# mateomarin/two_towers

Measured on AMD Instinct MI355X. Metric: training pairs/sec at global batch=8192, 1/2/4/8 GPUs; MRR@10 match, higher is better.
Workload: dtype bf16; 1 GPU; BASELINE configs[2]: EnhancedTwoTowerModel(300, 256), seq_len 64, batch 8192 per GPU, bf16, hard-negative mining k=5 + margin 0.2, dropout 0.1, Adam; global_batch=8192, seq_len=64, hidden=256, embedding_dim=300, parallelism=dp1, loss=hardneg_margin

## Files before the change

### include/tt_hip.h

```cpp
#ifndef TT_HIP_H
#define TT_HIP_H
#include <stdint.h>

#ifdef __cplusplus
extern "C" {
#endif

#define TT_OK 0
#define TT_EINVAL 1000
#define TT_DT_F32 0
#define TT_DT_BF16 1

const char* tt_version(void);
const char* tt_last_error(void);
int tt_set_option(const char* name, int value);
int tt_get_option(const char* name, int* value);

int tt_embed_gather(int dtype, const void* table, long vocab, int ep, const int32_t* ids, long n,
                    void* out, void* stream);

int tt_pack_rows(int dtype, const float* src, long n, int e, int ep, void* out, void* stream);
typedef struct {
  const float* src;
  const float* src2;
  void* dst;
  int rows, cols, dcols;
  long lds, ldd;
  int dst_bf16;
} tt_pack_job;
int tt_pack_multi(const tt_pack_job* jobs, int njobs, void* stream);

int tt_cast(int dtype, const float* x, long n, void* y, void* stream);

int tt_colsum(const float* x, long rows, int cols, long ld, float* out, int accumulate, void* stream);

typedef struct {
  const void* a[4];
  const void* b[4];
  void* c[4];
  const float* bias[4];
  int bshift[4];
  const void* a_hi[4];
  int a_split;
  uint32_t drop_row0;
} tt_gemm_batch;

int tt_gemm(int dtype, int out_dtype, int a_kouter, int b_kouter, int m, int n, int k,
            const tt_gemm_batch* batch, int nbatch, long lda, long ldb, long ldc, float alpha,
            int beta_accum, int relu, int seq_t, uint32_t drop_seed, float drop_p, int splits,
            float* splitk_ws, void* stream);
long tt_gemm_ws_size(int m, int n, int nbatch, int splits);
int tt_gemm_pick_splits(int m, int n, int k, int nbatch);

typedef struct {
  const void* g;
  const void* whh;
  const float* bhn;
  void* y;
  void* x1;
// ... 136 lines not shown
```

### two_towers_amd/_lib.py

```python
from __future__ import annotations

import contextlib
import ctypes
import os
from ctypes import POINTER, c_float, c_int, c_long, c_uint32, c_void_p

import torch

_HERE = os.path.dirname(os.path.abspath(__file__))
LIB_PATH = os.environ.get("TT_HIP_LIB", os.path.join(_HERE, "lib", "libtt_hip.so"))

DT_F32 = 0
DT_BF16 = 1
TT_EINVAL = 1000


class TTError(RuntimeError):
    pass


class GruTimeoutError(TTError):
    """A column-split GRU forward launch gave up waiting for one of its member workgroups
    (tt_gru_fwd's status word): that launch's outputs are invalid."""


class GemmBatch(ctypes.Structure):
    _fields_ = [
        ("a", c_void_p * 4),
        ("b", c_void_p * 4),
        ("c", c_void_p * 4),
        ("bias", c_void_p * 4),
        ("bshift", c_int * 4),
        ("a_hi", c_void_p * 4),
        ("a_split", c_int),
        ("drop_row0", c_uint32),
    ]


class PackJob(ctypes.Structure):
    _fields_ = [
        ("src", c_void_p),
        ("src2", c_void_p),
        ("dst", c_void_p),
        ("rows", c_int),
        ("cols", c_int),
        ("dcols", c_int),
        ("lds", c_long),
        ("ldd", c_long),
        ("dst_bf16", c_int),
    ]


class GruFwdRec(ctypes.Structure):
    _fields_ = [
        ("g", c_void_p), ("whh", c_void_p), ("bhn", c_void_p), ("y", c_void_p), ("x1", c_void_p),
        ("save", c_void_p), ("hstate", c_void_p), ("dir", c_int), ("drop_seed", c_uint32),
        ("drop_col0", c_int), ("drop_row0", c_uint32),
    ]


class GruInferRec(ctypes.Structure):
    _fields_ = [
        ("g", c_void_p), ("whh", c_void_p), ("bhn", c_void_p), ("y", c_void_p), ("hfinal", c_void_p),
        ("scratch", c_void_p), ("dir", c_int),
# ... 189 lines not shown
```

### two_towers_amd/csrc/tt_api.h

```cpp
#pragma once
#include <hip/hip_runtime.h>
#include <stdio.h>
#include <string.h>

#include "../../include/tt_hip.h"

namespace tt {
void set_error(const char* fmt, ...);

enum Opt {
  OPT_GRU_STEP,
  OPT_GRU_DEPTH,
  OPT_GRU_BWD_ROWS,
  OPT_GRU_BWD_BIG,
  OPT_GRU_BWD_STREAMS,
  OPT_GEMM_PERSIST,
  OPT_GEMM_A3,
  OPT_GEMM_REGSTAGE,
  OPT_GEMM_STREAM_OUT,
  OPT_HN_GEMM,
  OPT_GRU_BWD_PERSIST,
  OPT_GRU_FWD_STEP_ROWS,
  OPT_INFONCE_FLASH,
  OPT_HN_MAP,
// ... 3 lines not shown
  OPT_GRU_XC_SKIP,
  OPT_GRU_XC_SPINS,
  OPT_GRU_BWD_SKEW,
  OPT_GRU_FWD_SKEW,
  OPT_GEMM_BRES,
  OPT_GRU_XC_COOP,
  OPT_GEMM_BUF,
  OPT_GEMM_ORDER,
  OPT_GRU_STEP_RING,
  OPT_GRU_FWD_XS,
  OPT_HN_SCAN_GEMM,
  OPT_GEMM_IEPI,
  OPT_BRES_ROWS,
  OPT_HN_SCAN_V,
  OPT_GEMM_W4,
  OPT_N
};
int opt(Opt o);
int tt_hn_scan_gemm(const void* q, long bq, const void* d, long nd, int h, long label_off, float* cm, long nch,
                    hipStream_t st);
}

#define TT_CHECK_ARG(cond, ...)            \
  do {                                     \
    if (!(cond)) {                         \
      tt::set_error(__VA_ARGS__);          \
      return TT_EINVAL;                    \
    }                                      \
  } while (0)

// ... 26 lines not shown
```

### two_towers_amd/csrc/tt_elem.hip

```cpp
#include <algorithm>

#include "tt_api.h"
#include "tt_common.h"

namespace {

__global__ __launch_bounds__(256) void embed_gather_kernel(const uint4* __restrict__ table, long vocab,
                                                           int cpr, const int32_t* __restrict__ ids,
                                                           long n, uint4* __restrict__ out) {
  const long total = n * cpr;
  for (long e = (long)blockIdx.x * 256 + threadIdx.x; e < total; e += (long)gridDim.x * 256) {
    const long row = e / cpr;
    const int c = (int)(e - row * cpr);
    const int id = ids[row];
    uint4 v = make_uint4(0, 0, 0, 0);
    if (id >= 0 && id < vocab) v = table[(long)id * cpr + c];
    out[e] = v;
  }
}

template <typename T>
__global__ __launch_bounds__(256) void pack_rows_kernel(const float* __restrict__ src, long n, int e, int ep,
                                                        T* __restrict__ out) {
  const long total = n * ep;
// ... 26 lines not shown
    out[c] = accumulate ? out[c] + t : t;
  }
}

__global__ __launch_bounds__(256) void sum_kernel(const float* __restrict__ x, long n, float scale,
                                                  float* __restrict__ out) {
  __shared__ float part[4];
  float s = 0.f;
  for (long i = threadIdx.x; i < n; i += 256) s += x[i];
  s = wave_sum(s);
  if ((threadIdx.x & 63) == 0) part[threadIdx.x >> 6] = s;
  __syncthreads();
  if (threadIdx.x == 0) out[0] = scale * (part[0] + part[1] + part[2] + part[3]);
}

struct PackArgs {
  tt_pack_job j[16];
  long start[17];
  int n;
};
__global__ __launch_bounds__(256) void pack_multi_kernel(PackArgs a) {
  const long total = a.start[a.n];
  for (long i = blockIdx.x * 256L + threadIdx.x; i < total; i += (long)gridDim.x * 256) {
    int k = 0;
    while (k + 1 < a.n && i >= a.start[k + 1]) ++k;
    const tt_pack_job& J = a.j[k];
    const long q = i - a.start[k];
    const int g4 = J.dcols / 4;
    const long r = q / g4;
    const int c = (int)(q - r * g4) * 4;
    float4 v = make_float4(0.f, 0.f, 0.f, 0.f);
    if (c < J.cols) {
      v = *reinterpret_cast<const float4*>(J.src + r * J.lds + c);
      if (J.src2) {
        const float4 w = *reinterpret_cast<const float4*>(J.src2 + r * J.lds + c);
        v.x += w.x; v.y += w.y; v.z += w.z; v.w += w.w;
      }
    }
    if (J.dst_bf16) {
      const uint2 o = make_uint2((uint32_t)f2bf(v.x) | ((uint32_t)f2bf(v.y) << 16),
                                 (uint32_t)f2bf(v.z) | ((uint32_t)f2bf(v.w) << 16));
      *reinterpret_cast<uint2*>(static_cast<bf16_t*>(J.dst) + r * J.ldd + c) = o;
// ... 25 lines not shown
}

extern "C" int tt_pack_rows(int dtype, const float* src, long n, int e, int ep, void* out, void* stream) {
  TT_CHECK_ARG(ep >= e, "tt_pack_rows: ep < e");
  if (n == 0) return 0;
  dim3 g(grid_for(n * ep));
  if (dtype == TT_DT_BF16)
    hipLaunchKernelGGL(pack_rows_kernel<bf16_t>, g, dim3(256), 0, (hipStream_t)stream, src, n, e, ep, (bf16_t*)out);
  else
    hipLaunchKernelGGL(pack_rows_kernel<float>, g, dim3(256), 0, (hipStream_t)stream, src, n, e, ep, (float*)out);
  TT_CHECK_LAUNCH("pack_rows_kernel");
  return 0;
}

extern "C" int tt_pack_multi(const tt_pack_job* jobs, int njobs, void* stream) {
  TT_CHECK_ARG(njobs >= 0 && njobs <= 16 && (njobs == 0 || jobs), "tt_pack_multi: njobs %d not in [0,16]", njobs);
  PackArgs a{};
  a.n = njobs;
  a.start[0] = 0;
  for (int k = 0; k < njobs; ++k) {
    const tt_pack_job& J = jobs[k];
    TT_CHECK_ARG(J.src && J.dst && J.rows >= 0 && J.cols >= 0 && J.dcols >= J.cols, "tt_pack_multi: job %d", k);
    TT_CHECK_ARG(J.cols % 4 == 0 && J.dcols % 4 == 0 && J.lds % 4 == 0 && J.ldd % 4 == 0 && J.lds >= J.cols &&
                     J.ldd >= J.dcols,
                 "tt_pack_multi: job %d: cols, dcols and leading dimensions must be multiples of 4", k);
    const bool src_ok = ((uintptr_t)J.src | (uintptr_t)J.src2) % 16 == 0;
    TT_CHECK_ARG(src_ok && (uintptr_t)J.dst % (J.dst_bf16 ? 8 : 16) == 0, "tt_pack_multi: job %d: misaligned operand", k);
    a.j[k] = J;
    a.start[k + 1] = a.start[k] + (long)J.rows * (J.dcols / 4);
  }
  if (a.start[njobs] == 0) return 0;
  hipLaunchKernelGGL(pack_multi_kernel, dim3(grid_for(a.start[njobs], 256, 4096)), dim3(256), 0, (hipStream_t)stream, a);
  TT_CHECK_LAUNCH("pack_multi_kernel");
  return 0;
}

extern "C" int tt_cast(int dtype, const float* x, long n, void* y, void* stream) {
  if (n == 0) return 0;
  dim3 g(grid_for(n));
  if (dtype == TT_DT_BF16)
    hipLaunchKernelGGL(cast_kernel<bf16_t>, g, dim3(256), 0, (hipStream_t)stream, x, n, (bf16_t*)y);
  else
    hipLaunchKernelGGL(cast_kernel<float>, g, dim3(256), 0, (hipStream_t)stream, x, n, (float*)y);
  TT_CHECK_LAUNCH("cast_kernel");
// ... 22 lines not shown
```

### two_towers_amd/csrc/tt_gemm.hip

```cpp
#include <float.h>
#include <stdarg.h>
#include <stdlib.h>

#include <atomic>
#include <type_traits>

#include "tt_api.h"
#include "tt_gemm_core.h"

namespace tt {
static thread_local char g_err[512];
void set_error(const char* fmt, ...) {
  va_list ap;
  va_start(ap, fmt);
  vsnprintf(g_err, sizeof(g_err), fmt, ap);
  va_end(ap);
}
}

namespace tt {
namespace {
struct OptDef {
  const char* name;
  const char* env;
// ... 4 lines not shown
    {"gru_bwd_rows", "TT_GRU_BWD_ROWS", 0},     {"gru_bwd_big", "TT_GRU_BWD_BIG", 1},
    {"gru_bwd_streams", "TT_GRU_BWD_STREAMS", 2}, {"gemm_persist", "TT_GEMM_PERSIST", 1},
    {"gemm_a3", "TT_GEMM_A3", 1},                 {"gemm_regstage", "TT_GEMM_REGSTAGE", 0},
    {"gemm_stream_out", "TT_GEMM_STREAM_OUT", 1}, {"hn_gemm", "TT_HN_GEMM", 0},
    {"gru_bwd_persist", "TT_GRU_BWD_PERSIST", 1}, {"gru_fwd_step_rows", "TT_GRU_FWD_STEP_ROWS", 0},
    {"infonce_flash", "TT_INFONCE_FLASH", 1},     {"hn_map", "TT_HN_MAP", 2},
    {"gemm_skew", "TT_GEMM_SKEW", 0},             {"gemm_persist_maxk", "TT_GEMM_PERSIST_MAXK", 24},
    {"gru_fwd_xc", "TT_GRU_FWD_XC", 1},           {"gru_xc_skip", "TT_GRU_XC_SKIP", 0},
    {"gru_xc_spins", "TT_GRU_XC_SPINS", 22},      {"gru_bwd_skew", "TT_GRU_BWD_SKEW", 14},
    {"gru_fwd_skew", "TT_GRU_FWD_SKEW", 0},       {"gemm_bres", "TT_GEMM_BRES", 1},
    {"gru_xc_coop", "TT_GRU_XC_COOP", 0},         {"gemm_buf", "TT_GEMM_BUF", 1},
    {"gemm_order", "TT_GEMM_ORDER", 0},           {"gru_step_ring", "TT_GRU_STEP_RING", 4},
    {"gru_fwd_xs", "TT_GRU_FWD_XS", 1},           {"hn_scan_gemm", "TT_HN_SCAN_GEMM", 0},
    {"gemm_iepi", "TT_GEMM_IEPI", 1},             {"bres_rows", "TT_BRES_ROWS", 32},
    {"hn_scan_v", "TT_HN_SCAN_V", 5},             {"gemm_w4", "TT_GEMM_W4", 0},
};
struct OptTable {
  std::atomic<int> v[OPT_N];
  OptTable() {
    for (int i = 0; i < OPT_N; ++i) {
      const char* e = getenv(kOpts[i].env);
      v[i].store(e && *e ? atoi(e) : kOpts[i].dflt, std::memory_order_relaxed);
    }
  }
};
OptTable& opts() {
  static OptTable t;
  return t;
}
int find_opt(const char* name) {
// ... 23 lines not shown
namespace {

struct GemmArgs {
  const void* a[4];
  const void* b[4];
  void* c[4];
  const float* bias[4];
  int bshift[4];
  const void* a_hi[4];
  int a_split;
  long lda, ldb, ldc;
  int M, N, K;
  int splits, kt_per_split;
  float alpha;
  int beta, relu, seq_t;
  uint32_t drop_seed, drop_thresh, drop_row0;
  float drop_inv_keep;
  long part_stride;
  int vec_ok;
  int force_regstage;
  int skew;
  int bias_vec_ok;
  int stream_out;
  int walk_g, walk_x;
  int nbatch;
  float* cm;
  long nch, label_off;
};

constexpr int BM = 128, BN = 128;

// ... 126 lines not shown
      if (gm < g.M && gn < g.N) {
        float v[8];
#pragma unroll
        for (int e = 0; e < 8; ++e) v[e] = L[rl * CLD + cg + e];
        const bool full = gn + 8 <= g.N && g.vec_ok;
        if (partial) {
          float* dst = P + (long)gm * ldc + gn;
          if (full) st8(dst, v);
          else
            for (int e = 0; e < 8 && gn + e < g.N; ++e) dst[e] = v[e];
        } else {
#pragma unroll
          for (int e = 0; e < 8; ++e) {
            float x = v[e] * g.alpha + bv[e];
            if (g.relu) x = fmaxf(x, 0.f);
            if (g.drop_thresh) x *= tt_dropout_scale(g.drop_seed, g.drop_row0 + (uint32_t)gm, gn + e, g.drop_thresh, g.drop_inv_keep);
            v[e] = x;
          }
          TO* dst = C + (long)gm * ldc + gn;
          if (full) {
            if (g.beta) {
              float o[8];
              ld8(dst, o);
#pragma unroll
              for (int e = 0; e < 8; ++e) v[e] += o[e];
            }
            if (g.stream_out)
              st8_sc1(crs, (int)(((long)(gm - m0) * ldc + (gn - n0)) * (long)sizeof(TO)), v, (TO*)nullptr);
            else
              st8(dst, v);
          } else {
// ... 2 lines not shown
              if (g.beta) x += Elt<TO>::ld(dst + e);
              Elt<TO>::st(dst + e, x);
            }
          }
        }
      }
    }
    __syncthreads();
  }
}

template <typename TO>
constexpr int EPI_STORES = sizeof(TO) == 2 ? 16 : 32;

template <typename TO, int MI = -1, int NI = -1>
TT_DEV void epi_direct(const GemmArgs& g, const f32x4 (&acc)[8][4], TO* C, const float* bias, int m0, int n0,
                       int wm, int wn, bool full) {
  constexpr int I0 = MI < 0 ? 0 : 4 * MI, I1 = MI < 0 ? 8 : 4 * MI + 4;
  constexpr int JP0 = NI < 0 ? 0 : NI, JP1 = NI < 0 ? 2 : NI + 1;
  const int lane = threadIdx.x & 63, q = lane >> 4, lr = lane & 15;
  float bv[4][4];
#pragma unroll
  for (int j = 0; j < 4; ++j)
#pragma unroll
    for (int e = 0; e < 4; ++e) bv[j][e] = 0.f;
  if (bias) {
#pragma unroll
    for (int j = 2 * JP0; j < 2 * JP1; ++j) {
      const int c = n0 + wn + 16 * j + 4 * q;
      if (full && g.bias_vec_ok) {
        const float4 b4 = *reinterpret_cast<const float4*>(bias + c);
        bv[j][0] = b4.x; bv[j][1] = b4.y; bv[j][2] = b4.z; bv[j][3] = b4.w;
// ... 3 lines not shown
      }
    }
  }
#ifdef TT_DIAG
  if (g.force_regstage == 9) {
    float sum = 0.f;
#pragma unroll
    for (int i = 0; i < 8; ++i)
#pragma unroll
      for (int j = 0; j < 4; ++j) sum += acc[i][j][0] + acc[i][j][3] + bv[j][0];
    if (sum == 12345.f) C[0] = (TO)0;
    return;
  }
#endif
  const __amdgpu_buffer_rsrc_t crs = tt_rsrc(C + (long)m0 * g.ldc + n0);
  auto fin = [&](float x, float b, int gm, int gn) {
    x = x * g.alpha + b;
    if (g.relu) x = fmaxf(x, 0.f);
    if (g.drop_thresh) x *= tt_dropout_scale(g.drop_seed, g.drop_row0 + (uint32_t)gm, gn, g.drop_thresh, g.drop_inv_keep);
    return x;
  };
  auto put = [&](int gm, int gn, uint4 v) {
#ifdef TT_DIAG
    if (g.force_regstage == 10) {
      *reinterpret_cast<uint4*>(C + (long)(gm & 63) * g.ldc + gn) = v;
      return;
    }
#endif
    const int off = (int)(((long)(gm - m0) * g.ldc + (gn - n0)) * (long)sizeof(TO));
    if (g.stream_out == 2) st16_buf_aux<2>(crs, off, v);
    else if (g.stream_out == 3) st16_buf_aux<17>(crs, off, v);
    else if (g.stream_out) st16_sc1(crs, off, v);
    else *reinterpret_cast<uint4*>(C + (long)gm * g.ldc + gn) = v;
  };
// ... 340 lines not shown
    } else {
      return ttg::KOPlain<T>{B, g.ldb, t.n0, q < qend ? g.N - t.n0 : 0};
    }
  };
#ifdef TT_DIAG
  if constexpr (A3) {
    if (g.force_regstage == 11) {
      f32x4 acc[8][4];
#pragma unroll
      for (int i = 0; i < 8; ++i)
#pragma unroll
        for (int j = 0; j < 4; ++j) acc[i][j] = f32x4{(float)i, (float)j, 1.f, 2.f};
      for (int q = qbeg; q < qend; q += qstep) {
        const TileId t = decode(q);
        const bool full = t.m0 + 256 <= g.M && t.n0 + 256 <= g.N && g.vec_ok;
        epi_direct<TO>(g, acc, static_cast<TO*>(g.c[t.bi]), g.bias[t.bi], t.m0, t.n0, wm, wn, full);
      }
      return;
    }
  }
#endif
  auto la = loader_a(qbeg);
  auto lb = loader_b(qbeg);
  typename L8::template Half<AKO, decltype(la)> pa0, pa1;
  typename L8::template Half<BKO, decltype(lb)> pb0, pb1;
  pa0.init(la, 0, nk, g.K, 0);
  pa1.init(la, 0, nk, g.K, 128);
  pb0.init(lb, 0, nk, g.K, 0);
  pb1.init(lb, 0, nk, g.K, 128);
  if constexpr (A3) {
    pa0.issue(0, base);
// ... 160 lines not shown
      }
      ra_off -= nk;
      rb_off -= nk;
      if constexpr (HN) {
        epi_chunkmax(g, acc, cur_t.m0, cur_t.n0, wm, wn);
        epi_full = __builtin_amdgcn_readfirstlane((int)(cur_t.m0 + 256 <= g.M && cur_t.n0 + 256 <= 64 * g.nch)) != 0;
        continue;
      }
      const bool full = cur_t.m0 + 256 <= g.M && cur_t.n0 + 256 <= g.N && g.vec_ok;
      if constexpr (IEPI) {
        prev_t = cur_t;
        have_prev = true;
        epi_full = __builtin_amdgcn_readfirstlane((int)full) != 0;
        continue;
      }
      epi_direct<TO>(g, acc, static_cast<TO*>(g.c[cur_t.bi]), g.bias[cur_t.bi], cur_t.m0, cur_t.n0, wm, wn, full);
      epi_full = __builtin_amdgcn_readfirstlane((int)full) != 0;
      continue;
    }
    for (int r = 0; r < (A3 ? 0 : nk); ++r, ++git) {
      const int cs = git & 1;
      const uint32_t cur = base + cs * L8::SLOT, nxt = base + (cs ^ 1) * L8::SLOT;
      const char* ia = lds + cs * L8::SLOT + wr * L8::HALF;
      const char* ib = lds + cs * L8::SLOT + (2 + bh) * L8::HALF;
      if (r + 1 == nk) {
        la = loader_a(qn);
        pa0.init(la, 0, nk, g.K, 0);
        pa1.init(la, 0, nk, g.K, 128);
        ra_off = nk;
      }
#pragma unroll
// ... 56 lines not shown
      asm volatile("s_waitcnt lgkmcnt(0)" ::: "memory");
      __builtin_amdgcn_s_barrier();
#pragma unroll
      for (int k = 0; k < 2; ++k) {
        const int rl = rlo + 16 * k;
        const int gm = m0 + p * 32 + rl, gn = n0 + cg;
        if (gm < g.M && gn < g.N) {
          float v[8];
          const float4 x0 = *reinterpret_cast<const float4*>(stg + rl * 256 + cg);
          const float4 x1 = *reinterpret_cast<const float4*>(stg + rl * 256 + cg + 4);
          v[0] = x0.x; v[1] = x0.y; v[2] = x0.z; v[3] = x0.w; v[4] = x1.x; v[5] = x1.y; v[6] = x1.z; v[7] = x1.w;
#pragma unroll
          for (int e = 0; e < 8; ++e) {
            float x = v[e] * g.alpha + bv[e];
            if (g.relu) x = fmaxf(x, 0.f);
            if (g.drop_thresh) x *= tt_dropout_scale(g.drop_seed, g.drop_row0 + (uint32_t)gm, gn + e, g.drop_thresh, g.drop_inv_keep);
            v[e] = x;
          }
          TO* dst = C + (long)gm * g.ldc + gn;
          if (gn + 8 <= g.N && g.vec_ok) {
            if (g.stream_out)
              st8_sc1(crs, (int)(((long)(gm - m0) * g.ldc + (gn - n0)) * (long)sizeof(TO)), v, (TO*)nullptr);
            else
              st8(dst, v);
          } else {
            for (int e = 0; e < 8 && gn + e < g.N; ++e) Elt<TO>::st(dst + e, v[e]);
          }
        }
      }
      __builtin_amdgcn_s_barrier();
    }
// ... 341 lines not shown
  }
  if constexpr (std::is_same<T, bf16_t>::value && std::is_same<TO, bf16_t>::value) {
    if (tt::opt(tt::OPT_GEMM_W4) && !akout && !bkout && !shift && g.splits == 1 && !g.beta && !g.relu &&
        !g.drop_thresh && g.alpha == 1.f && g.force_regstage == 0 && g.M % 256 == 0 && g.N % 256 == 0 && g.K % 64 == 0 &&
        g.K >= 32 && g.vec_ok && g.bias_vec_ok && (g.lda * 2) % 16 == 0 && (g.ldb * 2) % 16 == 0 &&
        256L * g.lda * 2 < (1L << 31) && 256L * g.ldb * 2 < (1L << 31) && 256L * g.ldc * 2 < (1L << 31)) {
      const int ntm = g.M / 256, ntn = g.N / 256;
      if (tt::opt(tt::OPT_GEMM_W4) == 2)
        hipLaunchKernelGGL(gemm_w4<true>, dim3((unsigned)(ntm * ntn * nbatch)), dim3(256), 0, st, g, ntm, ntn);
      else
        hipLaunchKernelGGL(gemm_w4<false>, dim3((unsigned)(ntm * ntn * nbatch)), dim3(256), 0, st, g, ntm, ntn);
      TT_CHECK_LAUNCH("gemm_w4");
      return 0;
    }
  }
  if (dma && persist_ok && !shift && (g.force_regstage == 0 || g.force_regstage >= 9) && g.splits == 1 && !g.beta && nk >= 2 && nk <= tt::opt(tt::OPT_GEMM_PERSIST_MAXK) && t256 >= 512 &&
      use_big(g.M, g.N, t256))
    return launch_persist<T, TO>(akout, bkout, shift, g, (int)t256, buf, st);
  if (dma && g.force_regstage != 2 && use_big(g.M, g.N, t256)) {
    if (tt::opt(tt::OPT_GEMM_A3) && buf)
      return launch_t<T, TO, 256, 256, 2, 4, true, true, true>(akout, bkout, shift, g, t256, st);
    if (tt::opt(tt::OPT_GEMM_A3)) return launch_t<T, TO, 256, 256, 2, 4, true, true>(akout, bkout, shift, g, t256, st);
    return launch_t<T, TO, 256, 256, 2, 4, true>(akout, bkout, shift, g, t256, st);
  }
  const long t128 = (long)tt_ceil_div(g.M, 128) * tt_ceil_div(g.N, 128) * nbatch * g.splits;
  if (dma) return launch_t<T, TO, 128, 128, 2, 2, true>(akout, bkout, shift, g, t128, st);
  return launch_t<T, TO, 128, 128, 2, 2, false>(akout, bkout, shift, g, t128, st);
}

}

// ... 82 lines not shown
    g.a_hi[b] = batch->a_hi[b];
    if (batch->a_split > 0)
      TT_CHECK_ARG(batch->a_hi[b] && (uintptr_t)batch->a_hi[b] % 16 == 0, "tt_gemm: a_hi[%d] null or misaligned", b);
    if (batch->bshift[b] != 0) shift = true;
  }
  TT_CHECK_ARG(!shift || (b_kouter && seq_t > 0), "tt_gemm: bshift needs b_kouter and seq_t");
  TT_CHECK_ARG(batch->a_split >= 0 && (batch->a_split == 0 || (a_kouter && batch->a_split % (16 / esz) == 0)),
               "tt_gemm: a_split %d needs a_kouter and a 16-byte multiple", batch->a_split);
  g.a_split = batch->a_split;
  g.lda = lda; g.ldb = ldb; g.ldc = ldc;
  g.M = m; g.N = n; g.K = k;
  g.alpha = alpha; g.beta = beta_accum; g.relu = relu; g.seq_t = seq_t;
  g.force_regstage = tt::opt(tt::OPT_GEMM_REGSTAGE);
  g.nbatch = nbatch;
  g.skew = tt::opt(tt::OPT_GEMM_SKEW);
  g.drop_seed = drop_seed;
  g.drop_row0 = batch->drop_row0;
  g.drop_thresh = drop_p > 0.f ? (uint32_t)(drop_p * 16777216.0f + 0.5f) : 0u;
  g.drop_inv_keep = drop_p > 0.f ? 1.0f / (1.0f - drop_p) : 1.0f;
  const int nk = tt_ceil_div((long)k * esz, 128);
  if (splits > nk) splits = nk > 0 ? nk : 1;
  g.kt_per_split = nk > 0 ? tt_ceil_div(nk, splits) : 1;
  splits = nk > 0 ? tt_ceil_div(nk, g.kt_per_split) : 1;
  g.splits = splits;
  {
    const int osz = out_dtype == TT_DT_BF16 ? 2 : 4;
    bool ok = (ldc * osz) % 16 == 0;
    for (int b = 0; b < nbatch; ++b) ok = ok && ((uintptr_t)batch->c[b] % 16 == 0);
    g.vec_ok = ok;
    bool bok = true;
    for (int b = 0; b < nbatch; ++b) bok = bok && ((uintptr_t)batch->bias[b] % 16 == 0);
    g.bias_vec_ok = bok;
// ... 34 lines not shown
```

### two_towers_amd/ops.py

```python
from __future__ import annotations

import ctypes
from typing import Sequence

import torch

from . import _lib
from ._lib import GemmBatch, call, dtype_code, ptr, stream_ptr


def _esz(dt: torch.dtype) -> int:
    return 2 if dt == torch.bfloat16 else 4


def pad_cols(e: int, dt: torch.dtype) -> int:
    epc = 128 // _esz(dt)
    return (e + epc - 1) // epc * epc


def gemm(a: Sequence[torch.Tensor], b: Sequence[torch.Tensor], c: Sequence[torch.Tensor], *, m: int, n: int,
         k: int, lda: int, ldb: int, ldc: int, a_kouter: bool, b_kouter: bool, dtype: torch.dtype,
         out_dtype: torch.dtype, bias: Sequence[torch.Tensor | None] | None = None,
         bshift: Sequence[int] | None = None, alpha: float = 1.0, accumulate: bool = False,
         relu: bool = False, seq_t: int = 0, drop_seed: int = 0, drop_p: float = 0.0, drop_row0: int = 0,
         splits: int | None = None, a_hi: Sequence[torch.Tensor] | None = None, a_split: int = 0):
    nb = len(a)
    assert 1 <= nb <= 4 and len(b) == nb and len(c) == nb
    bt = GemmBatch()
    for i in range(nb):
        assert a[i].dtype == dtype and b[i].dtype == dtype, (a[i].dtype, b[i].dtype, dtype)
        assert c[i].dtype == out_dtype, (c[i].dtype, out_dtype)
        bt.a[i] = a[i].data_ptr()
        bt.b[i] = b[i].data_ptr()
        bt.c[i] = c[i].data_ptr()
        bt.bias[i] = bias[i].data_ptr() if bias is not None and bias[i] is not None else None
        bt.bshift[i] = bshift[i] if bshift is not None else 0
        if a_split:
            bt.a_hi[i] = a_hi[i].data_ptr()
    bt.a_split = a_split
    bt.drop_row0 = drop_row0 & 0xFFFFFFFF
    lib = _lib.load()
    if splits is None:
        splits = lib.tt_gemm_pick_splits(m, n, k, nb)
    ws = None
    if splits > 1 and not relu and drop_p == 0.0:
        ws = torch.empty(lib.tt_gemm_ws_size(m, n, nb, splits), dtype=torch.float32, device=c[0].device)
    else:
        splits = 1
    call("tt_gemm", dtype_code(dtype), dtype_code(out_dtype), int(a_kouter), int(b_kouter), m, n, k,
         ctypes.byref(bt), nb, lda, ldb, ldc, alpha, int(accumulate), int(relu), seq_t, drop_seed & 0xFFFFFFFF,
         drop_p, splits, ptr(ws), stream_ptr(c[0].device))


def embed_gather(table: torch.Tensor, ids: torch.Tensor, out: torch.Tensor):
    assert ids.dtype == torch.int32 and ids.is_contiguous()
    assert table.dim() == 2 and out.shape[-1] == table.shape[1] and out.dtype == table.dtype
    call("tt_embed_gather", dtype_code(table.dtype), table.data_ptr(), table.shape[0], table.shape[1],
         ids.data_ptr(), ids.numel(), out.data_ptr(), stream_ptr(out.device))


def pack_rows(src: torch.Tensor, out: torch.Tensor):
    assert src.dtype == torch.float32 and src.is_contiguous()
    e = src.shape[-1]
    n = src.numel() // e
    call("tt_pack_rows", dtype_code(out.dtype), src.data_ptr(), n, e, out.shape[-1], out.data_ptr(),
         stream_ptr(out.device))
# ... 38 lines not shown
```

### two_towers_amd/towers.py

```python
from __future__ import annotations

import ctypes
import os
import threading
from dataclasses import dataclass

import torch
import torch.nn.functional as F

from . import _lib, dist, ops, timing
from ._lib import GruBwdRec, GruFwdRec, GruInferRec, HeadBwdIO, HeadFwdIO, call, dtype_code, stream_ptr

PARAMS_PER_TOWER = 22
LN_EPS = 1e-5
HEAD_DT = torch.float32


def gru_param_names():
    names = []
    for layer in (0, 1):
        for sfx in ("", "_reverse"):
            for w in ("weight_ih", "weight_hh", "bias_ih", "bias_hh"):
                names.append(f"{w}_l{layer}{sfx}")
    return names
# ... 12 lines not shown
    dtype: torch.dtype
    drop_p: float
    head: str = "proj2"
    rank: int = 0

    @property
    def nparams(self) -> int:
        return PARAMS_PER_TOWER if self.head == "proj2" else len(GRU_NAMES)


_PACK_ONE = os.environ.get("TT_PACK_TORCH", "0") == "0"


class _Packed:

    def __init__(self, p, cfg: TowerCfg, Ep: int):
        dt, H, E = cfg.dtype, cfg.H, cfg.E
        g = dict(zip(GRU_NAMES, p[:16]))
        hd = dict(zip(HEAD_NAMES, p[16:]))
        self.wih = []
        self.bias = []
        self.whh = []
        self.bhn = []
        if _PACK_ONE and dt == torch.bfloat16 and E % 4 == 0 and H % 4 == 0 and all(
                t.is_contiguous() and t.dtype == torch.float32 and t.data_ptr() % 16 == 0 for t in p[:16]):
            self._pack_bf16(g, H, E, Ep, p[0].device)
        else:
            self._pack_torch(g, H, E, Ep, dt)
        if cfg.head == "none":
            return
        self.w1 = hd["0.weight"].float().contiguous()
        self.b1 = hd["0.bias"].float().contiguous()
        self.ln_g = hd["1.weight"].float().contiguous()
        self.ln_b = hd["1.bias"].float().contiguous()
        self.w2 = hd["3.weight"].float().contiguous()
        self.b2 = hd["3.bias"].float().contiguous()

    def _pack_bf16(self, g, H, E, Ep, dev):
        jobs = (_lib.PackJob * 16)()
        nj = 0

        def job(src, dst, rows, cols, dcols, lds, ldd, bf16, src2=None):
            nonlocal nj
            j = jobs[nj]
            j.src, j.src2, j.dst = src, src2, dst
            j.rows, j.cols, j.dcols, j.lds, j.ldd, j.dst_bf16 = rows, cols, dcols, lds, ldd, int(bf16)
            nj += 1
        for layer in (0, 1):
            K = E if layer == 0 else 2 * H
            Kp = Ep if layer == 0 else K
            w = _alloc((6 * H, Kp), torch.bfloat16, dev)
            b = _alloc((6 * H,), torch.float32, dev)
            whh = []
            for d, sfx in enumerate(("", "_reverse")):
                job(g[f"weight_ih_l{layer}{sfx}"].data_ptr(), w.data_ptr() + d * 3 * H * Kp * 2, 3 * H, K, Kp, K, Kp, True)
                bi, bh = g[f"bias_ih_l{layer}{sfx}"], g[f"bias_hh_l{layer}{sfx}"]
                job(bi.data_ptr(), b.data_ptr() + d * 3 * H * 4, 1, 2 * H, 2 * H, 2 * H, 2 * H, False, bh.data_ptr())
                job(bi.data_ptr() + 2 * H * 4, b.data_ptr() + (d * 3 + 2) * H * 4, 1, H, H, H, H, False)
                wh = _alloc((3 * H, H), torch.bfloat16, dev)
                job(g[f"weight_hh_l{layer}{sfx}"].data_ptr(), wh.data_ptr(), 3 * H, H, H, H, H, True)
                whh.append(wh)
            self.wih.append(w)
            self.bias.append(b)
            self.whh.append(whh)
            self.bhn.append([g[f"bias_hh_l{layer}{s}"][2 * H:] for s in ("", "_reverse")])
        call("tt_pack_multi", jobs, nj, stream_ptr(dev))

    def _pack_torch(self, g, H, E, Ep, dt):
        for layer in (0, 1):
            wf, wr = g[f"weight_ih_l{layer}"], g[f"weight_ih_l{layer}_reverse"]
# ... 5 lines not shown
            for sfx in ("", "_reverse"):
                bi, bh = g[f"bias_ih_l{layer}{sfx}"], g[f"bias_hh_l{layer}{sfx}"]
                bs.append(torch.cat([bi[: 2 * H] + bh[: 2 * H], bi[2 * H:]]))
            self.bias.append(torch.cat(bs).float().contiguous())
            self.whh.append([g[f"weight_hh_l{layer}{s}"].to(dt).contiguous() for s in ("", "_reverse")])
            self.bhn.append([g[f"bias_hh_l{layer}{s}"][2 * H:].float().contiguous() for s in ("", "_reverse")])


def _packed(p, cfg: TowerCfg, Ep: int, cache_ok: bool) -> _Packed:
    if not cache_ok:
        return _Packed(p, cfg, Ep)
    key = (cfg.dtype, cfg.H, cfg.head, Ep, tuple(t._version for t in p), tuple(t.data_ptr() for t in p))
    hit = getattr(p[0], "_tt_pack", None)
    if hit is not None and hit[0] == key:
        return hit[1]
    pk = _Packed(p, cfg, Ep)
    p[0]._tt_pack = (key, pk)
    return pk


def _alloc(shape, dt, dev):
    return torch.empty(shape, dtype=dt, device=dev)


_status_lock = threading.Lock()
_status_pending: list = []
_step_guard: dict = {}
_guard_reset: set = set()


def step_guard(dev) -> torch.Tensor:
# ... 432 lines not shown

        def layer1_wgrads():
            dWih1, dWhh1 = _weight_grads(cfg, B, T, dG1, Xl1, 2 * H, 2 * H, Y1)
            _layer_grads(gl, 1, E, Ep, dWih1, dWhh1, dbih1, dbhh1)
            if red is not None:
                _reduce_into(red, gl, head_grads)

        main = torch.cuda.current_stream(dev)
        side = _wgrad_stream(dev) if WGRAD_OVERLAP else None
        if side is None:
            layer1_wgrads()
        dY0 = [_alloc((B * T, 2 * H), dt, dev) for _ in range(n)]
        esz = 2 if dt == torch.bfloat16 else 4
        with timing.region("dgrad_l1", 1, 2.0 * B * T * 2 * H * 6 * H * n,
                           float(n * esz * (B * T * 6 * H + B * T * 2 * H))):
            if X1 is None:
                ops.gemm(dG1, [p.wih[1] for p in packs], dY0, m=B * T, n=2 * H, k=6 * H, lda=8 * H, ldb=2 * H,
                         ldc=2 * H, a_kouter=False, b_kouter=True, dtype=dt, out_dtype=dt)
            else:
                for ti in range(n):
                    ops.gemm([dG1[ti]], [packs[ti].wih[1]], [dY0[ti]], m=B * T, n=2 * H, k=6 * H, lda=8 * H,
                             ldb=2 * H, ldc=2 * H, a_kouter=False, b_kouter=True, dtype=dt, out_dtype=dt,
                             drop_seed=ctx.seeds[ti], drop_p=cfg.drop_p, drop_row0=cfg.rank * B * T)
        if side is not None:
            side.wait_stream(main)
            for t in (*dG1, *Xl1, *Y1, *[g for hg in head_grads for g in hg], *[x for b in dbih1 for x in b],
                      *[x for b in dbhh1 for x in b]):
                t.record_stream(side)
            with torch.cuda.stream(side):
                layer1_wgrads()
        del dG1
        dG0, dbih0, dbhh0 = _gru_layer_bwd(cfg, 0, B, T, S0, Y0, dY0, None, packs)
        del dY0
        dWih0, dWhh0 = _weight_grads(cfg, B, T, dG0, X0, Ep, Ep, Y0, kr=E)
        gl0 = [{} for _ in range(n)]
        _layer_grads(gl0, 0, E, Ep, dWih0, dWhh0, dbih0, dbhh0)
        if side is not None:
            main.wait_stream(side)
# ... 48 lines not shown
```

Baseline: 155,700 pairs/s.

## Pre-transpose layer-1 input weights so dgrad GEMM runs NT through persistent kernel

Adds a transposed pack mode to the multi-job pack kernel and stores a bf16 transposed copy of layer-1 W_ih during training packing. The layer-1 dgrad GEMM then uses the non-k-outer B layout, which can take the persistent GEMM path; a new option raises the persistent max-K for bf16 NT aligned shapes. Per-batch dropout seeds and row offsets let the dropout dgrad GEMMs be issued per tower with their own seeds. This costs an extra transpose pack and weight copy each step and more kernel argument state.

```diff
diff --git a/include/tt_hip.h b/include/tt_hip.h
--- a/include/tt_hip.h
+++ b/include/tt_hip.h
@@ -27,6 +27,7 @@
   int rows, cols, dcols;
   long lds, ldd;
   int dst_bf16;
+  int transpose;
 } tt_pack_job;
 int tt_pack_multi(const tt_pack_job* jobs, int njobs, void* stream);
 
@@ -42,7 +43,8 @@
   int bshift[4];
   const void* a_hi[4];
   int a_split;
-  uint32_t drop_row0;
+  uint32_t drop_seed[4];
+  uint32_t drop_row0[4];
 } tt_gemm_batch;
 
 int tt_gemm(int dtype, int out_dtype, int a_kouter, int b_kouter, int m, int n, int k,
diff --git a/two_towers_amd/_lib.py b/two_towers_amd/_lib.py
--- a/two_towers_amd/_lib.py
+++ b/two_towers_amd/_lib.py
@@ -33,7 +33,8 @@
         ("bshift", c_int * 4),
         ("a_hi", c_void_p * 4),
         ("a_split", c_int),
-        ("drop_row0", c_uint32),
+        ("drop_seed", c_uint32 * 4),
+        ("drop_row0", c_uint32 * 4),
     ]
 
 
@@ -48,6 +49,7 @@
         ("lds", c_long),
         ("ldd", c_long),
         ("dst_bf16", c_int),
+        ("transpose", c_int),
     ]
 
 
diff --git a/two_towers_amd/csrc/tt_api.h b/two_towers_amd/csrc/tt_api.h
--- a/two_towers_amd/csrc/tt_api.h
+++ b/two_towers_amd/csrc/tt_api.h
@@ -41,6 +41,7 @@
   OPT_BRES_ROWS,
   OPT_HN_SCAN_V,
   OPT_GEMM_W4,
+  OPT_GEMM_PERSIST_NT_MAXK,
   OPT_N
 };
 int opt(Opt o);
diff --git a/two_towers_amd/csrc/tt_elem.hip b/two_towers_amd/csrc/tt_elem.hip
--- a/two_towers_amd/csrc/tt_elem.hip
+++ b/two_towers_amd/csrc/tt_elem.hip
@@ -64,11 +64,41 @@
   if (threadIdx.x == 0) out[0] = scale * (part[0] + part[1] + part[2] + part[3]);
 }
 
+constexpr int PACK_JOBS = 24;
 struct PackArgs {
-  tt_pack_job j[16];
-  long start[17];
+  tt_pack_job j[PACK_JOBS];
+  long start[PACK_JOBS + 1];
   int n;
 };
+__device__ __forceinline__ void pack_transposed(const tt_pack_job& J, long q) {
+  const int tc = (J.cols + 15) / 16;
+  const long t = q >> 6;
+  const int l = (int)(q & 63);
+  const long r = (t / tc) * 64 + (l >> 2) * 4;
+  const int c = (int)(t % tc) * 16 + (l & 3) * 4;
+  if (r >= J.rows || c >= J.cols) return;
+  float v[4][4];
+#pragma unroll
+  for (int e = 0; e < 4; ++e) {
+    float4 x = *reinterpret_cast<const float4*>(J.src + (r + e) * J.lds + c);
+    if (J.src2) {
+      const float4 w = *reinterpret_cast<const float4*>(J.src2 + (r + e) * J.lds + c);
+      x.x += w.x; x.y += w.y; x.z += w.z; x.w += w.w;
+    }
+    v[e][0] = x.x; v[e][1] = x.y; v[e][2] = x.z; v[e][3] = x.w;
+  }
+#pragma unroll
+  for (int f = 0; f < 4; ++f) {
+    if (J.dst_bf16) {
+      const uint2 o = make_uint2((uint32_t)f2bf(v[0][f]) | ((uint32_t)f2bf(v[1][f]) << 16),
+                                 (uint32_t)f2bf(v[2][f]) | ((uint32_t)f2bf(v[3][f]) << 16));
+      *reinterpret_cast<uint2*>(static_cast<bf16_t*>(J.dst) + (c + f) * J.ldd + r) = o;
+    } else {
+      *reinterpret_cast<float4*>(static_cast<float*>(J.dst) + (c + f) * J.ldd + r) =
+          make_float4(v[0][f], v[1][f], v[2][f], v[3][f]);
+    }
+  }
+}
 __global__ __launch_bounds__(256) void pack_multi_kernel(PackArgs a) {
   const long total = a.start[a.n];
   for (long i = blockIdx.x * 256L + threadIdx.x; i < total; i += (long)gridDim.x * 256) {
@@ -76,6 +106,10 @@
     while (k + 1 < a.n && i >= a.start[k + 1]) ++k;
     const tt_pack_job& J = a.j[k];
     const long q = i - a.start[k];
+    if (J.transpose) {
+      pack_transposed(J, q);
+      continue;
+    }
     const int g4 = J.dcols / 4;
     const long r = q / g4;
     const int c = (int)(q - r * g4) * 4;
@@ -131,7 +165,8 @@
 }
 
 extern "C" int tt_pack_multi(const tt_pack_job* jobs, int njobs, void* stream) {
-  TT_CHECK_ARG(njobs >= 0 && njobs <= 16 && (njobs == 0 || jobs), "tt_pack_multi: njobs %d not in [0,16]", njobs);
+  TT_CHECK_ARG(njobs >= 0 && njobs <= PACK_JOBS && (njobs == 0 || jobs), "tt_pack_multi: njobs %d not in [0,%d]", njobs,
+               PACK_JOBS);
   PackArgs a{};
   a.n = njobs;
   a.start[0] = 0;
@@ -139,12 +174,15 @@
     const tt_pack_job& J = jobs[k];
     TT_CHECK_ARG(J.src && J.dst && J.rows >= 0 && J.cols >= 0 && J.dcols >= J.cols, "tt_pack_multi: job %d", k);
     TT_CHECK_ARG(J.cols % 4 == 0 && J.dcols % 4 == 0 && J.lds % 4 == 0 && J.ldd % 4 == 0 && J.lds >= J.cols &&
-                     J.ldd >= J.dcols,
+                     (J.transpose || J.ldd >= J.dcols),
                  "tt_pack_multi: job %d: cols, dcols and leading dimensions must be multiples of 4", k);
     const bool src_ok = ((uintptr_t)J.src | (uintptr_t)J.src2) % 16 == 0;
     TT_CHECK_ARG(src_ok && (uintptr_t)J.dst % (J.dst_bf16 ? 8 : 16) == 0, "tt_pack_multi: job %d: misaligned operand", k);
+    TT_CHECK_ARG(!J.transpose || (J.rows % 4 == 0 && J.dcols == J.cols && J.ldd >= J.rows),
+                 "tt_pack_multi: job %d: a transposed job needs rows %% 4 == 0, dcols == cols and ldd >= rows", k);
     a.j[k] = J;
-    a.start[k + 1] = a.start[k] + (long)J.rows * (J.dcols / 4);
+    a.start[k + 1] = a.start[k] + (J.transpose ? 64L * ((J.rows + 63) / 64) * ((J.cols + 15) / 16)
+                                               : (long)J.rows * (J.dcols / 4));
   }
   if (a.start[njobs] == 0) return 0;
   hipLaunchKernelGGL(pack_multi_kernel, dim3(grid_for(a.start[njobs], 256, 4096)), dim3(256), 0, (hipStream_t)stream, a);
diff --git a/two_towers_amd/csrc/tt_gemm.hip b/two_towers_amd/csrc/tt_gemm.hip
--- a/two_towers_amd/csrc/tt_gemm.hip
+++ b/two_towers_amd/csrc/tt_gemm.hip
@@ -42,6 +42,7 @@
     {"gru_fwd_xs", "TT_GRU_FWD_XS", 1},           {"hn_scan_gemm", "TT_HN_SCAN_GEMM", 0},
     {"gemm_iepi", "TT_GEMM_IEPI", 1},             {"bres_rows", "TT_BRES_ROWS", 32},
     {"hn_scan_v", "TT_HN_SCAN_V", 5},             {"gemm_w4", "TT_GEMM_W4", 0},
+    {"gemm_persist_nt_maxk", "TT_GEMM_PERSIST_NT_MAXK", 48},
 };
 struct OptTable {
   std::atomic<int> v[OPT_N];
@@ -95,7 +96,8 @@
   int splits, kt_per_split;
   float alpha;
   int beta, relu, seq_t;
-  uint32_t drop_seed, drop_thresh, drop_row0;
+  uint32_t drop_seed[4], drop_row0[4];
+  uint32_t drop_thresh;
   float drop_inv_keep;
   long part_stride;
   int vec_ok;
@@ -252,7 +254,7 @@
           for (int e = 0; e < 8; ++e) {
             float x = v[e] * g.alpha + bv[e];
             if (g.relu) x = fmaxf(x, 0.f);
-            if (g.drop_thresh) x *= tt_dropout_scale(g.drop_seed, g.drop_row0 + (uint32_t)gm, gn + e, g.drop_thresh, g.drop_inv_keep);
+            if (g.drop_thresh) x *= tt_dropout_scale(g.drop_seed[bi], g.drop_row0[bi] + (uint32_t)gm, gn + e, g.drop_thresh, g.drop_inv_keep);
             v[e] = x;
           }
           TO* dst = C + (long)gm * ldc + gn;
@@ -285,8 +287,8 @@
 constexpr int EPI_STORES = sizeof(TO) == 2 ? 16 : 32;
 
 template <typename TO, int MI = -1, int NI = -1>
-TT_DEV void epi_direct(const GemmArgs& g, const f32x4 (&acc)[8][4], TO* C, const float* bias, int m0, int n0,
-                       int wm, int wn, bool full) {
+TT_DEV void epi_direct(const GemmArgs& g, const f32x4 (&acc)[8][4], TO* C, const float* bias, int bi, int m0,
+                       int n0, int wm, int wn, bool full) {
   constexpr int I0 = MI < 0 ? 0 : 4 * MI, I1 = MI < 0 ? 8 : 4 * MI + 4;
   constexpr int JP0 = NI < 0 ? 0 : NI, JP1 = NI < 0 ? 2 : NI + 1;
   const int lane = threadIdx.x & 63, q = lane >> 4, lr = lane & 15;
@@ -320,10 +322,11 @@
   }
 #endif
   const __amdgpu_buffer_rsrc_t crs = tt_rsrc(C + (long)m0 * g.ldc + n0);
+  const uint32_t dseed = g.drop_seed[bi], drow0 = g.drop_row0[bi];
   auto fin = [&](float x, float b, int gm, int gn) {
     x = x * g.alpha + b;
     if (g.relu) x = fmaxf(x, 0.f);
-    if (g.drop_thresh) x *= tt_dropout_scale(g.drop_seed, g.drop_row0 + (uint32_t)gm, gn, g.drop_thresh, g.drop_inv_keep);
+    if (g.drop_thresh) x *= tt_dropout_scale(dseed, drow0 + (uint32_t)gm, gn, g.drop_thresh, g.drop_inv_keep);
     return x;
   };
   auto put = [&](int gm, int gn, uint4 v) {
@@ -694,7 +697,7 @@
       for (int q = qbeg; q < qend; q += qstep) {
         const TileId t = decode(q);
         const bool full = t.m0 + 256 <= g.M && t.n0 + 256 <= g.N && g.vec_ok;
-        epi_direct<TO>(g, acc, static_cast<TO*>(g.c[t.bi]), g.bias[t.bi], t.m0, t.n0, wm, wn, full);
+        epi_direct<TO>(g, acc, static_cast<TO*>(g.c[t.bi]), g.bias[t.bi], t.bi, t.m0, t.n0, wm, wn, full);
       }
       return;
     }
@@ -885,7 +888,8 @@
         epi_full = __builtin_amdgcn_readfirstlane((int)full) != 0;
         continue;
       }
-      epi_direct<TO>(g, acc, static_cast<TO*>(g.c[cur_t.bi]), g.bias[cur_t.bi], cur_t.m0, cur_t.n0, wm, wn, full);
+      epi_direct<TO>(g, acc, static_cast<TO*>(g.c[cur_t.bi]), g.bias[cur_t.bi], cur_t.bi, cur_t.m0, cur_t.n0, wm, wn,
+                     full);
       epi_full = __builtin_amdgcn_readfirstlane((int)full) != 0;
       continue;
     }
@@ -972,7 +976,7 @@
           for (int e = 0; e < 8; ++e) {
             float x = v[e] * g.alpha + bv[e];
             if (g.relu) x = fmaxf(x, 0.f);
-            if (g.drop_thresh) x *= tt_dropout_scale(g.drop_seed, g.drop_row0 + (uint32_t)gm, gn + e, g.drop_thresh, g.drop_inv_keep);
+            if (g.drop_thresh) x *= tt_dropout_scale(g.drop_seed[cur_t.bi], g.drop_row0[cur_t.bi] + (uint32_t)gm, gn + e, g.drop_thresh, g.drop_inv_keep);
             v[e] = x;
           }
           TO* dst = C + (long)gm * g.ldc + gn;
@@ -1344,7 +1348,12 @@
       return 0;
     }
   }
-  if (dma && persist_ok && !shift && (g.force_regstage == 0 || g.force_regstage >= 9) && g.splits == 1 && !g.beta && nk >= 2 && nk <= tt::opt(tt::OPT_GEMM_PERSIST_MAXK) && t256 >= 512 &&
+  int maxk = tt::opt(tt::OPT_GEMM_PERSIST_MAXK);
+  if constexpr (std::is_same<T, bf16_t>::value && std::is_same<TO, bf16_t>::value) {
+    if (!akout && !bkout && buf && tt::opt(tt::OPT_GEMM_A3) && g.M % 256 == 0 && g.N % 256 == 0 && g.vec_ok)
+      maxk = std::max(maxk, tt::opt(tt::OPT_GEMM_PERSIST_NT_MAXK));
+  }
+  if (dma && persist_ok && !shift && (g.force_regstage == 0 || g.force_regstage >= 9) && g.splits == 1 && !g.beta && nk >= 2 && nk <= maxk && t256 >= 512 &&
       use_big(g.M, g.N, t256))
     return launch_persist<T, TO>(akout, bkout, shift, g, (int)t256, buf, st);
   if (dma && g.force_regstage != 2 && use_big(g.M, g.N, t256)) {
@@ -1457,8 +1466,10 @@
   g.force_regstage = tt::opt(tt::OPT_GEMM_REGSTAGE);
   g.nbatch = nbatch;
   g.skew = tt::opt(tt::OPT_GEMM_SKEW);
-  g.drop_seed = drop_seed;
-  g.drop_row0 = batch->drop_row0;
+  for (int b = 0; b < nbatch; ++b) {
+    g.drop_seed[b] = drop_seed + batch->drop_seed[b];
+    g.drop_row0[b] = batch->drop_row0[b];
+  }
   g.drop_thresh = drop_p > 0.f ? (uint32_t)(drop_p * 16777216.0f + 0.5f) : 0u;
   g.drop_inv_keep = drop_p > 0.f ? 1.0f / (1.0f - drop_p) : 1.0f;
   const int nk = tt_ceil_div((long)k * esz, 128);
diff --git a/two_towers_amd/ops.py b/two_towers_amd/ops.py
--- a/two_towers_amd/ops.py
+++ b/two_towers_amd/ops.py
@@ -22,8 +22,9 @@
          k: int, lda: int, ldb: int, ldc: int, a_kouter: bool, b_kouter: bool, dtype: torch.dtype,
          out_dtype: torch.dtype, bias: Sequence[torch.Tensor | None] | None = None,
          bshift: Sequence[int] | None = None, alpha: float = 1.0, accumulate: bool = False,
-         relu: bool = False, seq_t: int = 0, drop_seed: int = 0, drop_p: float = 0.0, drop_row0: int = 0,
-         splits: int | None = None, a_hi: Sequence[torch.Tensor] | None = None, a_split: int = 0):
+         relu: bool = False, seq_t: int = 0, drop_seed: int | Sequence[int] = 0, drop_p: float = 0.0,
+         drop_row0: int | Sequence[int] = 0, splits: int | None = None,
+         a_hi: Sequence[torch.Tensor] | None = None, a_split: int = 0):
     nb = len(a)
     assert 1 <= nb <= 4 and len(b) == nb and len(c) == nb
     bt = GemmBatch()
@@ -38,7 +39,12 @@
         if a_split:
             bt.a_hi[i] = a_hi[i].data_ptr()
     bt.a_split = a_split
-    bt.drop_row0 = drop_row0 & 0xFFFFFFFF
+    seeds = [drop_seed] * nb if isinstance(drop_seed, int) else list(drop_seed)
+    row0s = [drop_row0] * nb if isinstance(drop_row0, int) else list(drop_row0)
+    assert len(seeds) == nb and len(row0s) == nb
+    for i in range(nb):
+        bt.drop_seed[i] = seeds[i] & 0xFFFFFFFF
+        bt.drop_row0[i] = row0s[i] & 0xFFFFFFFF
     lib = _lib.load()
     if splits is None:
         splits = lib.tt_gemm_pick_splits(m, n, k, nb)
@@ -48,8 +54,8 @@
     else:
         splits = 1
     call("tt_gemm", dtype_code(dtype), dtype_code(out_dtype), int(a_kouter), int(b_kouter), m, n, k,
-         ctypes.byref(bt), nb, lda, ldb, ldc, alpha, int(accumulate), int(relu), seq_t, drop_seed & 0xFFFFFFFF,
-         drop_p, splits, ptr(ws), stream_ptr(c[0].device))
+         ctypes.byref(bt), nb, lda, ldb, ldc, alpha, int(accumulate), int(relu), seq_t, 0, drop_p,
+         splits, ptr(ws), stream_ptr(c[0].device))
 
 
 def embed_gather(table: torch.Tensor, ids: torch.Tensor, out: torch.Tensor):
diff --git a/two_towers_amd/towers.py b/two_towers_amd/towers.py
--- a/two_towers_amd/towers.py
+++ b/two_towers_amd/towers.py
@@ -50,19 +50,22 @@
 
 class _Packed:
 
-    def __init__(self, p, cfg: TowerCfg, Ep: int):
+    def __init__(self, p, cfg: TowerCfg, Ep: int, train: bool = True):
         dt, H, E = cfg.dtype, cfg.H, cfg.E
         g = dict(zip(GRU_NAMES, p[:16]))
         hd = dict(zip(HEAD_NAMES, p[16:]))
         self.wih = []
+        self.wih_t = [None, None]
         self.bias = []
         self.whh = []
         self.bhn = []
         if _PACK_ONE and dt == torch.bfloat16 and E % 4 == 0 and H % 4 == 0 and all(
                 t.is_contiguous() and t.dtype == torch.float32 and t.data_ptr() % 16 == 0 for t in p[:16]):
-            self._pack_bf16(g, H, E, Ep, p[0].device)
+            self._pack_bf16(g, H, E, Ep, p[0].device, train)
         else:
             self._pack_torch(g, H, E, Ep, dt)
+            if train:
+                self.wih_t[1] = self.wih[1].t().contiguous()
         if cfg.head == "none":
             return
         self.w1 = hd["0.weight"].float().contiguous()
@@ -72,15 +75,16 @@
         self.w2 = hd["3.weight"].float().contiguous()
         self.b2 = hd["3.bias"].float().contiguous()
 
-    def _pack_bf16(self, g, H, E, Ep, dev):
-        jobs = (_lib.PackJob * 16)()
+    def _pack_bf16(self, g, H, E, Ep, dev, train=False):
+        jobs = (_lib.PackJob * 18)()
         nj = 0
 
-        def job(src, dst, rows, cols, dcols, lds, ldd, bf16, src2=None):
+        def job(src, dst, rows, cols, dcols, lds, ldd, bf16, src2=None, transpose=False):
             nonlocal nj
             j = jobs[nj]
             j.src, j.src2, j.dst = src, src2, dst
             j.rows, j.cols, j.dcols, j.lds, j.ldd, j.dst_bf16 = rows, cols, dcols, lds, ldd, int(bf16)
+            j.transpose = int(transpose)
             nj += 1
         for layer in (0, 1):
             K = E if layer == 0 else 2 * H
@@ -90,6 +94,11 @@
             whh = []
             for d, sfx in enumerate(("", "_reverse")):
                 job(g[f"weight_ih_l{layer}{sfx}"].data_ptr(), w.data_ptr() + d * 3 * H * Kp * 2, 3 * H, K, Kp, K, Kp, True)
+                if layer == 1 and train:
+                    if d == 0:
+                        self.wih_t[1] = _alloc((K, 6 * H), torch.bfloat16, dev)
+                    job(g[f"weight_ih_l{layer}{sfx}"].data_ptr(), self.wih_t[1].data_ptr() + d * 3 * H * 2, 3 * H, K, K, K,
+                        6 * H, True, transpose=True)
                 bi, bh = g[f"bias_ih_l{layer}{sfx}"], g[f"bias_hh_l{layer}{sfx}"]
                 job(bi.data_ptr(), b.data_ptr() + d * 3 * H * 4, 1, 2 * H, 2 * H, 2 * H, 2 * H, False, bh.data_ptr())
                 job(bi.data_ptr() + 2 * H * 4, b.data_ptr() + (d * 3 + 2) * H * 4, 1, H, H, H, H, False)
@@ -125,7 +134,7 @@
     hit = getattr(p[0], "_tt_pack", None)
     if hit is not None and hit[0] == key:
         return hit[1]
-    pk = _Packed(p, cfg, Ep)
+    pk = _Packed(p, cfg, Ep, train=False)
     p[0]._tt_pack = (key, pk)
     return pk
 
@@ -588,14 +597,15 @@
         esz = 2 if dt == torch.bfloat16 else 4
         with timing.region("dgrad_l1", 1, 2.0 * B * T * 2 * H * 6 * H * n,
                            float(n * esz * (B * T * 6 * H + B * T * 2 * H))):
+            wt = [p.wih_t[1] if p.wih_t[1] is not None else p.wih[1].t().contiguous() for p in packs]
+            kw = dict(m=B * T, n=2 * H, k=6 * H, lda=8 * H, ldb=6 * H, ldc=2 * H, a_kouter=False, b_kouter=False,
+                      dtype=dt, out_dtype=dt)
             if X1 is None:
-                ops.gemm(dG1, [p.wih[1] for p in packs], dY0, m=B * T, n=2 * H, k=6 * H, lda=8 * H, ldb=2 * H,
-                         ldc=2 * H, a_kouter=False, b_kouter=True, dtype=dt, out_dtype=dt)
+                ops.gemm(dG1, wt, dY0, **kw)
             else:
                 for ti in range(n):
-                    ops.gemm([dG1[ti]], [packs[ti].wih[1]], [dY0[ti]], m=B * T, n=2 * H, k=6 * H, lda=8 * H,
-                             ldb=2 * H, ldc=2 * H, a_kouter=False, b_kouter=True, dtype=dt, out_dtype=dt,
-                             drop_seed=ctx.seeds[ti], drop_p=cfg.drop_p, drop_row0=cfg.rank * B * T)
+                    ops.gemm([dG1[ti]], [wt[ti]], [dY0[ti]], drop_seed=ctx.seeds[ti], drop_p=cfg.drop_p,
+                             drop_row0=cfg.rank * B * T, **kw)
         if side is not None:
             side.wait_stream(main)
             for t in (*dG1, *Xl1, *Y1, *[g for hg in head_grads for g in hg], *[x for b in dbih1 for x in b],
```

Result: no change. 156,000 pairs/s (median of 6 runs) (+0.2%).
